# Edward-Sun/DIFUSCO

Measured on NVIDIA H100. Metric: TSP-500 graphs/sec, 50-step categorical denoise, higher is better.
Workload: dtype f32 (3-term bf16 split on wgmma, fp32 accumulate)

## Files before the change

difusco_b200/_cabi.py:

```python
import ctypes as C
import os

import numpy as np

HERE = os.path.dirname(os.path.abspath(__file__))
LIB_PATH = os.path.join(HERE, "libdifusco_b200.so")

DFB_OK, DFB_E_INVALID, DFB_E_CUDA, DFB_E_UNSUPPORTED, DFB_E_NOMEM = 0, -1, -2, -3, -4
CATEGORICAL, GAUSSIAN = 0, 1
EDGE_IMPL_TC, EDGE_IMPL_FP32, EDGE_IMPL_TC1 = 0, 1, 2
AGGREGATION = {"sum": 0, "mean": 1, "max": 2}

SYMBOLS = [
    "dfb_abi_version", "dfb_create", "dfb_destroy", "dfb_last_error", "dfb_set_aggregation",
    "dfb_set_edge_impl", "dfb_load_weights", "dfb_prepare_graph", "dfb_set_points",
    "dfb_encoder_forward", "dfb_denoise_step", "dfb_denoise", "dfb_denoise_record", "dfb_denoise_host",
    "dfb_launch_count", "dfb_profile_begin", "dfb_profile_end", "dfb_debug_edge_gemm", "dfb_debug_gnn_layer",
    "dfb_debug_phase_cycles", "dfb_debug_watchdog", "dfb_knn_graph", "dfb_set_graph_capture",
    "dfb_set_phase_timing", "dfb_tsp_merge_sparse", "dfb_tsp_merge_order", "dfb_two_opt", "dfb_write_heatmap_txt",
]

_lib = None


def lib():
  global _lib
  if _lib is not None:
    return _lib
  if not os.path.exists(LIB_PATH):
    raise RuntimeError(
        f"{LIB_PATH} not found: build it with `python -m difusco_b200.build` "
        "(difusco_b200 has no fallback path; the CUDA library is the product)")
  L = C.CDLL(LIB_PATH)
  vp, i32, i64, u64, f32 = C.c_void_p, C.c_int, C.c_int64, C.c_uint64, C.c_float
  L.dfb_abi_version.restype = i32
  L.dfb_create.argtypes = [C.POINTER(vp), i32]
  L.dfb_destroy.argtypes = [vp]
  L.dfb_last_error.argtypes = [vp]
  L.dfb_last_error.restype = C.c_char_p
  L.dfb_set_aggregation.argtypes = [vp, i32]
  L.dfb_set_edge_impl.argtypes = [vp, i32]
  L.dfb_load_weights.argtypes = [vp, i32, i32, i32, i32, i32, C.POINTER(C.c_char_p), C.POINTER(vp),
                                 C.POINTER(i64)]
  L.dfb_prepare_graph.argtypes = [vp, vp, i64, i64, i32, vp]
  L.dfb_set_points.argtypes = [vp, vp, vp]
  L.dfb_encoder_forward.argtypes = [vp, vp, f32, vp, vp]
  L.dfb_denoise_step.argtypes = [vp, i32, vp, f32, C.POINTER(f32), i32, vp, u64, i32, vp, vp, vp, vp]
  L.dfb_denoise.argtypes = [vp, i32, vp, i32, C.POINTER(C.c_int32), C.POINTER(f32),
                            C.POINTER(C.c_int32), vp, u64, vp]
  L.dfb_denoise_record.argtypes = [vp, i32, vp, i32, C.POINTER(C.c_int32), C.POINTER(f32), C.POINTER(C.c_int32), vp,
                                   u64, i32, C.POINTER(C.c_int32), vp, vp, vp, vp]
  L.dfb_denoise_host.argtypes = [vp, i32, vp, vp, i64, i64, i32, vp, i32, C.POINTER(C.c_int32),
                                 C.POINTER(f32), C.POINTER(C.c_int32), u64, vp, vp]
  L.dfb_launch_count.argtypes = [vp]
  L.dfb_launch_count.restype = i64
  L.dfb_profile_begin.argtypes = [vp]
  L.dfb_profile_end.argtypes = [vp, C.POINTER(C.c_double), C.POINTER(i64)]
  L.dfb_debug_edge_gemm.argtypes = [vp, i32, vp, vp, vp]
  L.dfb_debug_gnn_layer.argtypes = [vp, i32, f32, vp, vp, vp]
  L.dfb_debug_phase_cycles.argtypes = [vp, C.POINTER(C.c_uint64)]
  L.dfb_debug_watchdog.argtypes = [vp, C.POINTER(C.c_int)]
  L.dfb_set_graph_capture.argtypes = [vp, i32]
  L.dfb_set_phase_timing.argtypes = [vp, i32]
  L.dfb_knn_graph.argtypes = [vp, vp, i64, i32, i64, vp, vp]
  L.dfb_tsp_merge_sparse.argtypes = [vp, i64, vp, vp, i64, i32, vp, C.POINTER(i64)]
  L.dfb_tsp_merge_order.argtypes = [i64, vp, i64, vp, C.POINTER(i64)]
  L.dfb_two_opt.argtypes = [vp, vp, i64, vp, i64, i64, C.POINTER(i64), vp]
  L.dfb_write_heatmap_txt.argtypes = [C.c_char_p, i64, vp]
  for name in SYMBOLS:
    fn = getattr(L, name)
    if fn.restype is C.c_int and name not in ("dfb_abi_version",):
      fn.restype = i32
  _lib = L
  return L


class DfbError(RuntimeError):
  pass


def _raise(code, msg):
  msg = msg.decode() if isinstance(msg, bytes) else msg
  if code == DFB_E_INVALID:
    raise ValueError(msg)
  if code == DFB_E_UNSUPPORTED:
    raise NotImplementedError(msg)
  if code == DFB_E_NOMEM:
    raise MemoryError(msg)
  raise DfbError(msg)


MERGE_COMPLETE, MERGE_INCOMPLETE, MERGE_AMBIGUOUS = 0, 1, 2


def tsp_merge_sparse(points, heat, edge_index, mode=0):
  points = np.ascontiguousarray(points, dtype=np.float64)
  heat = np.ascontiguousarray(heat, dtype=np.float32).reshape(-1)
  edge_index = np.ascontiguousarray(edge_index, dtype=np.int64)
  n = points.shape[0]
  if edge_index.ndim != 2 or edge_index.shape[0] != 2 or edge_index.shape[1] != heat.shape[0]:
    raise ValueError("edge_index must be (2, E) with one heat value per edge")
  tour = np.empty(n + 1, dtype=np.int64)
  it = C.c_int64(0)
  rc = lib().dfb_tsp_merge_sparse(points.ctypes.data, n, heat.ctypes.data, edge_index.ctypes.data, heat.shape[0],
                                  int(mode), tour.ctypes.data, C.byref(it))
  if rc < 0:
    _raise(rc, "dfb_tsp_merge_sparse: invalid argument (n >= 3, indices inside [0, n), mode 0/1)")
  return rc, tour, it.value


def tsp_merge_order(n, order):
  order = np.ascontiguousarray(order, dtype=np.int64).reshape(-1)
  tour = np.empty(n + 1, dtype=np.int64)
  it = C.c_int64(0)
# ... 96 lines not shown
  def denoise(self, diffusion, xt_ptr, t1, consts, last, uniforms_ptr=None, seed=0, stream=0):
    steps, t1a, ca, la = self._sched_arrays(t1, consts, last)
    self._ck(lib().dfb_denoise(self._h, diffusion, xt_ptr, steps, t1a, ca, la, uniforms_ptr,
                               int(seed) & 0xFFFFFFFFFFFFFFFF, stream))

  def denoise_record(self, diffusion, xt_ptr, t1, consts, last, record_steps, rec_xt_ptr=None, rec_p_ptr=None,
                     rec_out_ptr=None, uniforms_ptr=None, seed=0, stream=0):
    steps, t1a, ca, la = self._sched_arrays(t1, consts, last)
    n_rec = len(record_steps)
    ra = (C.c_int32 * max(n_rec, 1))(*[int(x) for x in record_steps])
    self._ck(lib().dfb_denoise_record(self._h, diffusion, xt_ptr, steps, t1a, ca, la, uniforms_ptr,
                                      int(seed) & 0xFFFFFFFFFFFFFFFF, n_rec, ra, rec_xt_ptr, rec_p_ptr, rec_out_ptr,
                                      stream))

  def denoise_host(self, diffusion, points_ptr, edge_index_ptr, num_nodes, num_edges, gn_segments, xt0_ptr,
                   t1, consts, last, seed, heatmap_ptr, stream=0):
    steps, t1a, ca, la = self._sched_arrays(t1, consts, last)
    self._ck(lib().dfb_denoise_host(self._h, diffusion, points_ptr, edge_index_ptr, num_nodes, num_edges,
                                    gn_segments, xt0_ptr, steps, t1a, ca, la,
                                    int(seed) & 0xFFFFFFFFFFFFFFFF, heatmap_ptr, stream))

  def two_opt(self, points, tours, max_iterations, stream=0):
    points = np.ascontiguousarray(points, dtype=np.float64)
    tours = np.array(tours, dtype=np.int64, order="C", copy=True)
    if tours.ndim != 2 or tours.shape[1] != points.shape[0] + 1:
      raise ValueError("tours must be (batch, n + 1)")
    it = C.c_int64(0)
    self._ck(lib().dfb_two_opt(self._h, points.ctypes.data, points.shape[0], tours.ctypes.data, tours.shape[0],
                               int(max_iterations), C.byref(it), stream))
    return tours, it.value

  def knn_graph(self, points_ptr, num_nodes, k, node_offset, edge_index_ptr, stream=0):
    self._ck(lib().dfb_knn_graph(self._h, points_ptr, int(num_nodes), int(k), int(node_offset), edge_index_ptr, stream))

  def launch_count(self):
    return int(lib().dfb_launch_count(self._h))

  def profile_begin(self):
    self._ck(lib().dfb_profile_begin(self._h))

  def profile_end(self):
    ms, n = C.c_double(0), C.c_int64(0)
    self._ck(lib().dfb_profile_end(self._h, C.byref(ms), C.byref(n)))
    return ms.value, n.value

  def set_graph_capture(self, enabled):
    self._ck(lib().dfb_set_graph_capture(self._h, int(bool(enabled))))

  def debug_watchdog(self):
    out = (C.c_int * 4)()
    lib().dfb_debug_watchdog(self._h, out)
    return [int(x) for x in out]

  def set_phase_timing(self, enabled):
    self._ck(lib().dfb_set_phase_timing(self._h, int(bool(enabled))))

  def debug_phase_cycles(self):
    out = (C.c_uint64 * 32)()
    self._ck(lib().dfb_debug_phase_cycles(self._h, out))
    return [int(x) for x in out]

  def debug_edge_gemm(self, layer, e_in_ptr, acc_out_ptr, stream=0):
    self._ck(lib().dfb_debug_edge_gemm(self._h, layer, e_in_ptr, acc_out_ptr, stream))

  def debug_gnn_layer(self, layer, t, h_ptr, e_ptr, stream=0):
    self._ck(lib().dfb_debug_gnn_layer(self._h, int(layer), float(t), h_ptr, e_ptr, stream))
```

difusco_b200/csrc/dfb_api.cu:

```cuda
#include <cuda_runtime.h>
#include <math.h>
#include <stdio.h>
#include <stdlib.h>
#include <string.h>

#include <map>
#include <string>
#include <vector>

#include "../../include/difusco_b200.h"
#include "common.cuh"
#include "edge_layer_fp32.cuh"
#include "edge_layer_tc.cuh"
#include "kernels_small.cuh"
#include "knn.cuh"
#include "tsp_decode.cuh"

using namespace dfb;

static std::string g_create_error;

struct DevBuf {
  void* p = nullptr;
  size_t cap = 0;
// ... 938 lines not shown
  if (ms) *ms = tot;
  if (n) *n = (int64_t)(ctx->ev_used / 2);
  ctx->profiling = false;
  ctx->ev_used = 0;
  return DFB_OK;
}

extern "C" int dfb_debug_edge_gemm(dfb_ctx* ctx, int layer, const float* e_in, float* acc_out, void* stream_) {
  if (!ctx) return DFB_E_INVALID;
  cudaStream_t st = (cudaStream_t)stream_;
  CK(ctx, cudaSetDevice(ctx->device));
  if (!ctx->graph_ready) FAIL(ctx, DFB_E_INVALID, "dfb_prepare_graph must be called first");
  if (layer < 0 || layer >= ctx->L) FAIL(ctx, DFB_E_INVALID, "layer out of range");
  if (tc_launch_edge_layer(&ctx->tc, layer, const_cast<float*>(e_in), (const float*)ctx->uvab.p,
                           (float*)ctx->partials.p, ctx->g, ctx->layers[layer], nullptr, 0, 0, nullptr, ctx->lut, AGG_SUM,
                           edge_impl(ctx).nwg, false, acc_out, st))
    FAIL(ctx, DFB_E_CUDA, "tensor-core edge layer: %s", ctx->tc.err.c_str());
  ctx->launches++;
  return DFB_OK;
}

extern "C" int dfb_debug_gnn_layer(dfb_ctx* ctx, int layer, float t, float* h, float* e, void* stream_) {
  if (!ctx) return DFB_E_INVALID;
  cudaStream_t st = (cudaStream_t)stream_;
  CK(ctx, cudaSetDevice(ctx->device));
  if (!ctx->graph_ready) FAIL(ctx, DFB_E_INVALID, "dfb_prepare_graph must be called first");
  if (layer < 0 || layer >= ctx->L) FAIL(ctx, DFB_E_INVALID, "layer %d out of range for %d layers", layer, ctx->L);
  if (!is_device_ptr(h) || !is_device_ptr(e)) FAIL(ctx, DFB_E_INVALID, "h and e must be device pointers");
  int slot;
  int r = stage_acquire(ctx, &slot);
  if (r) return r;
  ctx->h_tvals[slot][0] = t;
  r = compute_tvecs(ctx, slot, 1, st);
  if (r) return r;
  CK(ctx, cudaEventRecord(ctx->stage_ev[slot], st));
  return run_layer(ctx, layer, h, e, nullptr, (const float*)ctx->tvec.p + (size_t)layer * H, 0, nullptr, st);
}

extern "C" int dfb_debug_phase_cycles(dfb_ctx* ctx, unsigned long long* out) {
  if (!ctx || !out) return DFB_E_INVALID;
  CK(ctx, cudaSetDevice(ctx->device));
  CK(ctx, cudaDeviceSynchronize());
  CK(ctx, cudaMemcpy(out, ctx->tc.phase_cycles, 32 * sizeof(unsigned long long), cudaMemcpyDeviceToHost));
  CK(ctx, cudaMemset(ctx->tc.phase_cycles, 0, 32 * sizeof(unsigned long long)));
  return DFB_OK;
}

extern "C" int dfb_debug_watchdog(dfb_ctx* ctx, int* out) {
  if (!ctx || !out || !ctx->tc.error_host) return DFB_E_INVALID;
  for (int i = 0; i < 4; ++i) out[i] = ((volatile int*)ctx->tc.error_host)[i];
  return DFB_OK;
}

extern "C" int dfb_knn_graph(dfb_ctx* ctx, const double* points, int64_t num_nodes, int k, int64_t node_offset,
                             int64_t* edge_index, void* stream_) {
  if (!ctx) return DFB_E_INVALID;
  cudaStream_t st = (cudaStream_t)stream_;
  CK(ctx, cudaSetDevice(ctx->device));
  if (num_nodes < 1 || k < 1 || k > num_nodes) FAIL(ctx, DFB_E_INVALID, "bad kNN size N=%lld K=%d", (long long)num_nodes, k);
  if ((size_t)num_nodes * sizeof(double) > 200 * 1024) FAIL(ctx, DFB_E_UNSUPPORTED, "kNN graph: N=%lld exceeds the shared-memory brute-force limit (25600)", (long long)num_nodes);
  const size_t smem = (size_t)num_nodes * sizeof(double) + (size_t)(num_nodes + 31) / 32 * sizeof(unsigned);
  if (!is_device_ptr(edge_index)) FAIL(ctx, DFB_E_INVALID, "edge_index must be a device pointer");
  const double* dp = points;
  if (!is_device_ptr(points)) {
    for (int64_t i = 0; i < 2 * num_nodes; ++i)
      if (!std::isfinite(points[i])) FAIL(ctx, DFB_E_INVALID, "kNN graph: non-finite coordinate of node %lld", (long long)(i / 2));
    ENS(ctx, ctx->d_points, (size_t)num_nodes * 2 * sizeof(double));
    CK(ctx, cudaMemcpyAsync(ctx->d_points.p, points, (size_t)num_nodes * 2 * sizeof(double), cudaMemcpyHostToDevice, st));
    dp = (const double*)ctx->d_points.p;
  }
  CK(ctx, cudaFuncSetAttribute(k_knn_bruteforce, cudaFuncAttributeMaxDynamicSharedMemorySize, (int)smem));
  k_knn_bruteforce<<<(int)num_nodes, 256, smem, st>>>(dp, (int)num_nodes, k, (long long*)edge_index, (long long)node_offset);
  CKL(ctx);
  return DFB_OK;
}

extern "C" int dfb_tsp_merge_sparse(const double* points, int64_t n, const float* heat, const int64_t* edge_index, int64_t E,
                                    int mode, int64_t* tour, int64_t* merge_iterations) {
  if (!points || !heat || !edge_index || !tour || !merge_iterations || n < 3 || n > 0x7fffffff / 2 || E < 0 || (mode != 0 && mode != 1))
    return DFB_E_INVALID;
  int r = tspmerge::merge_sparse(points, (int)n, heat, edge_index, E, mode, tour, merge_iterations);
  return r < 0 ? DFB_E_INVALID : r;
}

extern "C" int dfb_tsp_merge_order(int64_t n, const int64_t* order, int64_t count, int64_t* tour, int64_t* merge_iterations) {
  if (!order || !tour || !merge_iterations || n < 3 || n > 0x7fffffff / 2 || count < 0) return DFB_E_INVALID;
  int r = tspmerge::merge_order((int)n, order, count, tour, merge_iterations);
  return r < 0 ? DFB_E_INVALID : r;
}

extern "C" int dfb_two_opt(dfb_ctx* ctx, const double* points, int64_t n, int64_t* tours, int64_t batch, int64_t max_iterations,
                           int64_t* iterations_out, void* stream_) {
  if (!ctx) return DFB_E_INVALID;
  cudaStream_t st = (cudaStream_t)stream_;
  CK(ctx, cudaSetDevice(ctx->device));
  if (!points || !tours || !iterations_out) FAIL(ctx, DFB_E_INVALID, "two_opt: null argument");
  if (n < 3 || n > 46340 || batch < 1 || batch > 65535) FAIL(ctx, DFB_E_INVALID, "two_opt: bad size n=%lld batch=%lld (n in [3, 46340], batch in [1, 65535])", (long long)n, (long long)batch);
  const int N = (int)n, B = (int)batch;
  bool finite = true;
  for (int64_t k = 0; k < batch * (n + 1); ++k) {
    if (tours[k] < 0 || tours[k] >= n) FAIL(ctx, DFB_E_INVALID, "two_opt: tour entry %lld out of range", (long long)tours[k]);
    finite = finite && std::isfinite(points[2 * tours[k]]) && std::isfinite(points[2 * tours[k] + 1]);
  }
  if (!finite) {
    *iterations_out = 0;
    return DFB_OK;
// ... 79 lines not shown
```

difusco_b200/csrc/edge_layer_tc.cuh:

```cuda
#pragma once
#include <cuda.h>
#include <cuda_bf16.h>
#include <cuda_runtime.h>

#include <stdlib.h>

#include <string>

#include "common.cuh"
#include "edge_layer_fp32.cuh"

namespace dfb {

constexpr int WG_ROWS = 64;
constexpr int TC_KCH = 64;
constexpr int TC_B_BYTES = 256 * 128;
constexpr int TC_A_CHUNK = WG_ROWS * 128;
constexpr int TC_A_BYTES = 8 * TC_A_CHUNK;
constexpr int CONV_BATCH = 16;
constexpr int E4_BATCH = 16;

constexpr int W_LO_ROWS = H;
constexpr int W_MAT_ROWS = 2 * W_LO_ROWS;
constexpr int W_LAYER_ROWS = 6 * W_MAT_ROWS;
__host__ __device__ constexpr int w_row_C(int l) { return l * W_LAYER_ROWS; }
__host__ __device__ constexpr int w_row_O(int l) { return w_row_C(l) + W_MAT_ROWS; }
__host__ __device__ constexpr int w_row_UVAB(int l) { return w_row_C(l) + 2 * W_MAT_ROWS; }
__host__ __device__ constexpr int w_row_embed(int L, int which) { return L * W_LAYER_ROWS + which * W_MAT_ROWS; }
__host__ __device__ constexpr int w_arena_rows(int L) { return w_row_embed(L, 2); }

template <int NWG>
struct TcCfg {
  static_assert(NWG == 1 || NWG == 2, "one or two consumer warpgroups");
  static constexpr int TILE = NWG * WG_ROWS;
  static constexpr int THREADS = (NWG + 1) * 128;
  static constexpr int NSTAGE = (NWG == 1) ? 3 : 2;
  static constexpr int OFF_B = NWG * TC_A_BYTES;
  static constexpr int OFF_PRM = OFF_B + NSTAGE * TC_B_BYTES;
  static constexpr int OFF_ROW = OFF_PRM + 6 * H * 4;
  static constexpr int OFF_SRC = OFF_ROW + TILE * 4;
  static constexpr int OFF_BAR = OFF_SRC + TILE * 8;
  static constexpr int SMEM_BYTES = OFF_BAR + 2 * NSTAGE * 8;
  static constexpr int SMEM_ALLOC = SMEM_BYTES + 1024;
  static_assert(SMEM_ALLOC <= 232448, "shared memory budget (227 KB per block)");
};

struct TcParams {
  float* e;
  const float* uvab;
  float* partials;
  GraphDev g;
  LayerParams lp;
  const float* tvec;
  const float* xt_lut;
  const float* lut;
  const float* zero_row;
  float* debug_acc;
  const float* lin_in;
  float* lin_out;
  const float* lin_bias;
  int lin_rows;
  int lin_nb;
  int lin_w_row;
  int* error_flag;
  unsigned long long* phase_cycles;
  int write_e, e_zero, agg_mode;
  int w_row_base;
  int n_tiles;
};

__device__ __forceinline__ uint32_t smem_u32(const void* p) { return (uint32_t)__cvta_generic_to_shared(p); }

__device__ __forceinline__ void mbar_init(uint64_t* bar, uint32_t count) {
  asm volatile("mbarrier.init.shared::cta.b64 [%0], %1;" ::"r"(smem_u32(bar)), "r"(count) : "memory");
}
__device__ __forceinline__ void mbar_arrive(uint64_t* bar) {
  asm volatile("mbarrier.arrive.shared::cta.b64 _, [%0];" ::"r"(smem_u32(bar)) : "memory");
}
__device__ __forceinline__ void mbar_arrive_expect_tx(uint64_t* bar, uint32_t bytes) {
  asm volatile("mbarrier.arrive.expect_tx.shared::cta.b64 _, [%0], %1;" ::"r"(smem_u32(bar)), "r"(bytes) : "memory");
}
__device__ __forceinline__ void mbar_wait(uint64_t* bar, uint32_t parity, int* error_flag, int code) {
  const uint32_t addr = smem_u32(bar);
  uint32_t ok = 0;
#pragma unroll 1
  for (uint32_t spin = 0;; ++spin) {
    asm volatile(
        "{\n .reg .pred p;\n mbarrier.try_wait.parity.shared::cta.b64 p, [%1], %2, %3;\n selp.u32 %0, 1, 0, p;\n}"
        : "=r"(ok)
        : "r"(addr), "r"(parity), "r"(20000u)
        : "memory");
    if (ok) return;
    if (spin > 400000u) {
      if (error_flag) {
        error_flag[1] = (int)blockIdx.x;
        error_flag[2] = (int)parity;
        error_flag[3] = (int)threadIdx.x;
        atomicExch(error_flag, code);
      }
      __threadfence_system();
      __trap();
    }
  }
}
__device__ __forceinline__ void tma_load_2d(uint32_t dst, const CUtensorMap* map, uint64_t* bar, int c0, int c1) {
  asm volatile(
      "cp.async.bulk.tensor.2d.shared::cluster.global.mbarrier::complete_tx::bytes [%0], [%1, {%3, %4}], [%2];"
      ::"r"(dst), "l"(reinterpret_cast<uint64_t>(map)), "r"(smem_u32(bar)), "r"(c0), "r"(c1)
      : "memory");
}
__device__ __forceinline__ void fence_proxy_async() { asm volatile("fence.proxy.async.shared::cta;" ::: "memory"); }

__device__ __forceinline__ uint64_t wgmma_desc_sw128(uint32_t smem_addr) {
  return (uint64_t)((smem_addr >> 4) & 0x3fffu) | (1ull << 16) | (64ull << 32) | (1ull << 62);
}
__device__ __forceinline__ void wgmma_fence() { asm volatile("wgmma.fence.sync.aligned;" ::: "memory"); }
__device__ __forceinline__ void wgmma_commit() { asm volatile("wgmma.commit_group.sync.aligned;" ::: "memory"); }
template <int N>
__device__ __forceinline__ void wgmma_wait() { asm volatile("wgmma.wait_group.sync.aligned %0;" ::"n"(N) : "memory"); }
__device__ __forceinline__ void acc_fence(float (&d)[128]) {
#pragma unroll
  for (int i = 0; i < 128; ++i) asm volatile("" : "+f"(d[i])::"memory");
}
__device__ __forceinline__ void wgmma_bf16(float (&d)[128], uint64_t da, uint64_t db, uint32_t scale_d) {
  asm volatile(
      "{\n .reg .pred p;\n setp.ne.b32 p, %130, 0;\n"
      "wgmma.mma_async.sync.aligned.m64n256k16.f32.bf16.bf16 "
      "{%0, %1, %2, %3, %4, %5, %6, %7, %8, %9, %10, %11, %12, %13, %14, %15, "
      "%16, %17, %18, %19, %20, %21, %22, %23, %24, %25, %26, %27, %28, %29, %30, %31, "
      "%32, %33, %34, %35, %36, %37, %38, %39, %40, %41, %42, %43, %44, %45, %46, %47, "
      "%48, %49, %50, %51, %52, %53, %54, %55, %56, %57, %58, %59, %60, %61, %62, %63, "
      "%64, %65, %66, %67, %68, %69, %70, %71, %72, %73, %74, %75, %76, %77, %78, %79, "
      "%80, %81, %82, %83, %84, %85, %86, %87, %88, %89, %90, %91, %92, %93, %94, %95, "
      "%96, %97, %98, %99, %100, %101, %102, %103, %104, %105, %106, %107, %108, %109, %110, %111, "
      "%112, %113, %114, %115, %116, %117, %118, %119, %120, %121, %122, %123, %124, %125, %126, %127}, "
      "%128, %129, p, 1, 1, 0, 0;\n}"
      : "+f"(d[0]), "+f"(d[1]), "+f"(d[2]), "+f"(d[3]), "+f"(d[4]), "+f"(d[5]), "+f"(d[6]), "+f"(d[7]),
        "+f"(d[8]), "+f"(d[9]), "+f"(d[10]), "+f"(d[11]), "+f"(d[12]), "+f"(d[13]), "+f"(d[14]), "+f"(d[15]),
        "+f"(d[16]), "+f"(d[17]), "+f"(d[18]), "+f"(d[19]), "+f"(d[20]), "+f"(d[21]), "+f"(d[22]), "+f"(d[23]),
        "+f"(d[24]), "+f"(d[25]), "+f"(d[26]), "+f"(d[27]), "+f"(d[28]), "+f"(d[29]), "+f"(d[30]), "+f"(d[31]),
        "+f"(d[32]), "+f"(d[33]), "+f"(d[34]), "+f"(d[35]), "+f"(d[36]), "+f"(d[37]), "+f"(d[38]), "+f"(d[39]),
        "+f"(d[40]), "+f"(d[41]), "+f"(d[42]), "+f"(d[43]), "+f"(d[44]), "+f"(d[45]), "+f"(d[46]), "+f"(d[47]),
        "+f"(d[48]), "+f"(d[49]), "+f"(d[50]), "+f"(d[51]), "+f"(d[52]), "+f"(d[53]), "+f"(d[54]), "+f"(d[55]),
        "+f"(d[56]), "+f"(d[57]), "+f"(d[58]), "+f"(d[59]), "+f"(d[60]), "+f"(d[61]), "+f"(d[62]), "+f"(d[63]),
        "+f"(d[64]), "+f"(d[65]), "+f"(d[66]), "+f"(d[67]), "+f"(d[68]), "+f"(d[69]), "+f"(d[70]), "+f"(d[71]),
        "+f"(d[72]), "+f"(d[73]), "+f"(d[74]), "+f"(d[75]), "+f"(d[76]), "+f"(d[77]), "+f"(d[78]), "+f"(d[79]),
        "+f"(d[80]), "+f"(d[81]), "+f"(d[82]), "+f"(d[83]), "+f"(d[84]), "+f"(d[85]), "+f"(d[86]), "+f"(d[87]),
        "+f"(d[88]), "+f"(d[89]), "+f"(d[90]), "+f"(d[91]), "+f"(d[92]), "+f"(d[93]), "+f"(d[94]), "+f"(d[95]),
        "+f"(d[96]), "+f"(d[97]), "+f"(d[98]), "+f"(d[99]), "+f"(d[100]), "+f"(d[101]), "+f"(d[102]), "+f"(d[103]),
        "+f"(d[104]), "+f"(d[105]), "+f"(d[106]), "+f"(d[107]), "+f"(d[108]), "+f"(d[109]), "+f"(d[110]), "+f"(d[111]),
        "+f"(d[112]), "+f"(d[113]), "+f"(d[114]), "+f"(d[115]), "+f"(d[116]), "+f"(d[117]), "+f"(d[118]), "+f"(d[119]),
        "+f"(d[120]), "+f"(d[121]), "+f"(d[122]), "+f"(d[123]), "+f"(d[124]), "+f"(d[125]), "+f"(d[126]), "+f"(d[127])
      : "l"(da), "l"(db), "r"(scale_d));
}

__device__ __forceinline__ float sigmoid_mufu(float x) {
  float t, r;
  asm("ex2.approx.ftz.f32 %0, %1;" : "=f"(t) : "f"(-1.4426950408889634f * x));
  asm("rcp.approx.ftz.f32 %0, %1;" : "=f"(r) : "f"(1.0f + t));
  return r;
}
__device__ __forceinline__ void split4(float4 x, uint2& hi, uint2& lo) {
// ... 10 lines not shown
  __nv_bfloat162 h = __floats2bfloat162_rn(a, b);
  const float2 f = __bfloat1622float2(h);
  __nv_bfloat162 l = __floats2bfloat162_rn(a - f.x, b - f.y);
  hi = *reinterpret_cast<uint32_t*>(&h);
  lo = *reinterpret_cast<uint32_t*>(&l);
}
__device__ __forceinline__ uint32_t sw128_off(int r, int j) {
  return (uint32_t)((r >> 3) * 1024 + (r & 7) * 128 + ((j ^ (r & 7)) << 4));
}
__device__ __forceinline__ float quad_sum(float v) {
  v += __shfl_xor_sync(0xffffffffu, v, 1);
  return v + __shfl_xor_sync(0xffffffffu, v, 2);
}
__device__ __forceinline__ void swap_row_halves(float (&d)[128]) {
#pragma unroll
  for (int j = 0; j < 32; ++j) {
    const float x0 = d[4 * j], x1 = d[4 * j + 1];
    d[4 * j] = d[4 * j + 2];
    d[4 * j + 1] = d[4 * j + 3];
    d[4 * j + 2] = x0;
    d[4 * j + 3] = x1;
  }
}

enum {
  PH_TILES = 0,
  PH_TOTAL,
  PH_CONVERT,
  PH_G1_WAIT,
  PH_G1_MMA,
  PH_E1,
  PH_REDUCE,
  PH_LN,
  PH_G2_WAIT,
  PH_G2_MMA,
  PH_E4,
  PH_COUNT
};

template <int NWG, bool LIN, bool TIMED = false>
__device__ __forceinline__ void edge_layer_wg_body(const CUtensorMap& wmap, const TcParams& P) {
  using Cfg = TcCfg<NWG>;
  constexpr int NSTAGE = Cfg::NSTAGE;
  extern __shared__ unsigned char smem_raw[];
  unsigned char* smem = smem_raw + ((1024u - (smem_u32(smem_raw) & 1023u)) & 1023u);
  float* prm = reinterpret_cast<float*>(smem + Cfg::OFF_PRM);
  int* s_row = reinterpret_cast<int*>(smem + Cfg::OFF_ROW);
  const float** s_src = reinterpret_cast<const float**>(smem + Cfg::OFF_SRC);
  uint64_t* full = reinterpret_cast<uint64_t*>(smem + Cfg::OFF_BAR);
  uint64_t* empty = full + NSTAGE;

  const int warp = threadIdx.x >> 5, lane = threadIdx.x & 31;
  constexpr bool lin = LIN;
  const int loads_per_tile = (P.write_e ? 16 : 8) * NWG;

  if (threadIdx.x == 0) {
    for (int s = 0; s < NSTAGE; ++s) {
      mbar_init(&full[s], 1);
      mbar_init(&empty[s], 4);
    }
    asm volatile("fence.mbarrier_init.release.cluster;" ::: "memory");
    fence_proxy_async();
  }
  for (int i = threadIdx.x; i < H; i += Cfg::THREADS) {
    prm[i] = P.lp.ln_e_g[i];
    prm[H + i] = P.lp.ln_e_b[i];
    prm[2 * H + i] = P.tvec ? P.tvec[i] : 0.0f;
    prm[3 * H + i] = P.lp.ln_o_g[i];
    prm[4 * H + i] = P.lp.ln_o_b[i];
    prm[5 * H + i] = P.lp.b_O[i];
  }
  __syncthreads();
  const uint32_t smem_base = smem_u32(smem);

  if (warp >= 4 * NWG) {
    if constexpr (NWG == 2) asm volatile("setmaxnreg.dec.sync.aligned.u32 40;" ::: "memory");
    if (warp == 4 * NWG && lane == 0) {
      uint32_t u = 0;
      for (int tile = blockIdx.x; tile < P.n_tiles; tile += gridDim.x) {
        for (int i = 0; i < loads_per_tile; ++i, ++u) {
          const int s = u % NSTAGE;
          mbar_wait(&empty[s], ((u / NSTAGE) & 1) ^ 1, P.error_flag, 1);
          mbar_arrive_expect_tx(&full[s], TC_B_BYTES);
          const int row = (lin ? P.lin_w_row + (P.lin_nb == 4 ? (tile & 3) : 0) * W_MAT_ROWS
                               : P.w_row_base + (i >= 8 * NWG ? w_row_O(0) - w_row_C(0) : 0)) +
                          (i & 1) * W_LO_ROWS;
          tma_load_2d(smem_base + Cfg::OFF_B + s * TC_B_BYTES, &wmap, &full[s], ((i >> 1) & 3) * TC_KCH, row);
        }
      }
    }
    return;
  }

  if constexpr (NWG == 2) asm volatile("setmaxnreg.inc.sync.aligned.u32 232;" ::: "memory");
  const int wg = warp >> 2, wi = warp & 3, tid = threadIdx.x & 127;
  const int t4 = lane & 3;
  const int lr0 = wi * 16 + (lane >> 2);
  unsigned char* a_reg = smem + wg * TC_A_BYTES;
  const uint32_t a_base = smem_base + wg * TC_A_BYTES;
  float* msg = reinterpret_cast<float*>(a_reg);
  int* w_row = s_row + wg * WG_ROWS;
  const float** w_src = s_src + wg * WG_ROWS;
  auto wg_bar = [&] { asm volatile("bar.sync %0, 128;" ::"r"(1 + wg) : "memory"); };
  const int n_rows = lin ? P.lin_rows : P.g.E;
  uint32_t u = 0;
  float acc[128];

  auto turn_wait = [&] {
    if constexpr (NWG == 2) asm volatile("bar.sync %0, 256;" ::"r"(3 + wg) : "memory");
  };
  auto turn_pass = [&] {
    if constexpr (NWG == 2) asm volatile("bar.arrive %0, 256;" ::"r"(4 - wg) : "memory");
  };
  if (wg == 1) turn_pass();

  uint32_t t_mark = 0, t_start = 0;
  if constexpr (TIMED) t_start = t_mark = (uint32_t)clock();
  auto record = [&](int slot, uint32_t v) {
    if constexpr (TIMED) {
      if (tid == 0) atomicAdd(P.phase_cycles + slot, (unsigned long long)v);
    }
  };
  auto mark = [&](int slot) {
    if constexpr (TIMED) {
      const uint32_t now = (uint32_t)clock();
      record(slot, now - t_mark);
      t_mark = now;
    }
  };

  auto gemm = [&](int wait_slot, int mma_slot) {
    uint32_t waited = 0;
    turn_wait();
    if constexpr (TIMED) t_mark = (uint32_t)clock();
    acc_fence(acc);
    wgmma_fence();
    int s_prev = 0;
#pragma unroll
    for (int i = 0; i < 8; ++i, ++u) {
      const int s = u % NSTAGE;
      uint32_t w0 = 0;
      if constexpr (TIMED) w0 = (uint32_t)clock();
      mbar_wait(&full[s], (u / NSTAGE) & 1, P.error_flag, 2);
      if constexpr (TIMED) waited += (uint32_t)clock() - w0;
      const uint32_t b = smem_base + Cfg::OFF_B + s * TC_B_BYTES;
      const uint32_t ahi = a_base + (i >> 1) * 2 * TC_A_CHUNK, alo = ahi + TC_A_CHUNK;
#pragma unroll
      for (int ks = 0; ks < 4; ++ks) {
        const uint64_t db = wgmma_desc_sw128(b + ks * 32);
        wgmma_bf16(acc, wgmma_desc_sw128(ahi + ks * 32), db, (i | ks) ? 1u : 0u);
        if ((i & 1) == 0) wgmma_bf16(acc, wgmma_desc_sw128(alo + ks * 32), db, 1u);
      }
      wgmma_commit();
      if (i > 0) {
        wgmma_wait<1>();
        __syncwarp();
        if (lane == 0) mbar_arrive(&empty[s_prev]);
      }
      s_prev = s;
    }
    wgmma_wait<0>();
    acc_fence(acc);
    __syncwarp();
    if (lane == 0) mbar_arrive(&empty[s_prev]);
    turn_pass();
    if constexpr (TIMED) {
      const uint32_t now = (uint32_t)clock();
      record(wait_slot, waited);
      record(mma_slot, now - t_mark - waited);
      t_mark = now;
    }
  };

  for (int tile = blockIdx.x; tile < P.n_tiles; tile += gridDim.x) {
    record(PH_TILES, 1);
    const int row_tile = (lin && P.lin_nb == 4) ? (tile >> 2) : tile;
    const int s_base = row_tile * Cfg::TILE + wg * WG_ROWS;
    if (tid < WG_ROWS) {
      const int s = s_base + tid;
      const float* src = P.zero_row;
      int rw = -1;
      if (s < n_rows && lin) {
        src = P.lin_in + (size_t)s * H;
      } else if (s < n_rows) {
        rw = P.g.row[s];
        if (P.e_zero) src = P.zero_row;
        else if (P.xt_lut) src = P.lut + ((P.xt_lut[P.g.perm ? P.g.perm[s] : s] != 0.0f) ? H : 0);
        else src = P.e + (size_t)s * H;
      }
      w_row[tid] = rw;
      w_src[tid] = src;
    }
    wg_bar();

#pragma unroll 1
    for (int it0 = 0; it0 < 32; it0 += CONV_BATCH) {
      float4 x[CONV_BATCH];
#pragma unroll
      for (int q = 0; q < CONV_BATCH; ++q) {
        const int item = (it0 + q) * 128 + tid;
        x[q] = __ldcg(reinterpret_cast<const float4*>(w_src[item >> 6]) + (item & 63));
      }
#pragma unroll
      for (int q = 0; q < CONV_BATCH; ++q) {
        const int item = (it0 + q) * 128 + tid;
        const int rr = item >> 6, k4 = item & 63;
        uint2 hi, lo;
        split4(x[q], hi, lo);
        const uint32_t off = (k4 >> 4) * 2 * TC_A_CHUNK + sw128_off(rr, (k4 & 15) >> 1) + (k4 & 1) * 8;
        *reinterpret_cast<uint2*>(a_reg + off) = hi;
        *reinterpret_cast<uint2*>(a_reg + off + TC_A_CHUNK) = lo;
      }
    }
    fence_proxy_async();
    wg_bar();
    mark(PH_CONVERT);
    gemm(PH_G1_WAIT, PH_G1_MMA);

    const int sa = s_base + lr0, sb = sa + 8;
    const bool va = sa < n_rows, vb = sb < n_rows;
    if (lin || P.debug_acc) {
      const int nb = (lin && P.lin_nb == 4) ? (tile & 3) : 0;
      const int ostride = lin ? P.lin_nb * H : H;
      float* out = lin ? P.lin_out + nb * H : P.debug_acc;
#pragma unroll
      for (int h = 0; h < 2; ++h) {
        const int s = h ? sb : sa;
        if (!(h ? vb : va)) continue;
#pragma unroll
// ... 97 lines not shown
      mean = quad_sum(sum) * (1.0f / H);
      q = 0.f;
#pragma unroll
      for (int j = 0; j < 32; ++j) {
        const float d0 = acc[4 * j] - mean, d1 = acc[4 * j + 1] - mean;
        q = fmaf(d0, d0, fmaf(d1, d1, q));
      }
      rstd = rsqrtf(quad_sum(q) * (1.0f / H) + LN_EPS);
      const int r = lr0 + 8 * h;
#pragma unroll
      for (int j = 0; j < 32; ++j) {
        const int c = 8 * j + 2 * t4;
        const float2 g = *reinterpret_cast<const float2*>(prm + 3 * H + c);
        const float2 b = *reinterpret_cast<const float2*>(prm + 4 * H + c);
        const float z0 = fmaf((acc[4 * j] - mean) * rstd, g.x, b.x);
        const float z1 = fmaf((acc[4 * j + 1] - mean) * rstd, g.y, b.y);
        uint32_t hi, lo;
        split2(z0 * sigmoid_mufu(z0), z1 * sigmoid_mufu(z1), hi, lo);
        const uint32_t off = (j >> 3) * 2 * TC_A_CHUNK + sw128_off(r, j & 7) + 4 * t4;
        *reinterpret_cast<uint32_t*>(a_reg + off) = hi;
        *reinterpret_cast<uint32_t*>(a_reg + off + TC_A_CHUNK) = lo;
      }
      swap_row_halves(acc);
    }
    fence_proxy_async();
    wg_bar();
    mark(PH_LN);
    gemm(PH_G2_WAIT, PH_G2_MMA);

#pragma unroll
    for (int h = 0; h < 2; ++h) {
      if (!(h ? vb : va)) continue;
      const float* src = h ? src_b : src_a;
      float* dst = P.e + (size_t)(h ? sb : sa) * H;
#pragma unroll
      for (int j0 = 0; j0 < 32; j0 += E4_BATCH) {
        float2 ein[E4_BATCH];
#pragma unroll
        for (int q = 0; q < E4_BATCH; ++q) ein[q] = __ldcg(reinterpret_cast<const float2*>(src + 8 * (j0 + q) + 2 * t4));
#pragma unroll
        for (int q = 0; q < E4_BATCH; ++q) {
          const int j = j0 + q, c = 8 * j + 2 * t4;
          const float2 bo = *reinterpret_cast<const float2*>(prm + 5 * H + c);
          __stcg(reinterpret_cast<float2*>(dst + c),
                 make_float2((ein[q].x + acc[4 * j + 2 * h]) + bo.x, (ein[q].y + acc[4 * j + 2 * h + 1]) + bo.y));
        }
      }
    }
    mark(PH_E4);
  }
  if constexpr (TIMED) record(PH_TOTAL, (uint32_t)clock() - t_start);
}

__global__ void __launch_bounds__(TcCfg<2>::THREADS, 1)
k_edge_layer_wg2(const __grid_constant__ CUtensorMap wmap, const TcParams P) {
  edge_layer_wg_body<2, false>(wmap, P);
}
__global__ void __launch_bounds__(TcCfg<2>::THREADS, 1)
k_edge_layer_wg2_timed(const __grid_constant__ CUtensorMap wmap, const TcParams P) {
  edge_layer_wg_body<2, false, true>(wmap, P);
}
__global__ void __launch_bounds__(TcCfg<1>::THREADS, 1)
k_edge_layer_wg1(const __grid_constant__ CUtensorMap wmap, const TcParams P) {
  edge_layer_wg_body<1, false>(wmap, P);
}
__global__ void __launch_bounds__(TcCfg<2>::THREADS, 1)
k_linear_wg2(const __grid_constant__ CUtensorMap wmap, const TcParams P) {
  edge_layer_wg_body<2, true>(wmap, P);
}

struct TcState {
  std::string err;
  int num_sms = 0;
  CUtensorMap wmap;
  bool bound = false;
  float* zero_row = nullptr;
  int* error_flag = nullptr;
  int* error_host = nullptr;
  unsigned long long* phase_cycles = nullptr;

  TcState() = default;
  TcState(const TcState&) = delete;
  TcState& operator=(const TcState&) = delete;
  ~TcState() {
    if (zero_row) cudaFree(zero_row);
    if (error_host) cudaFreeHost(error_host);
    if (phase_cycles) cudaFree(phase_cycles);
  }
};

typedef CUresult (*PFN_encodeTiled)(CUtensorMap*, CUtensorMapDataType, cuuint32_t, void*, const cuuint64_t*,
                                    const cuuint64_t*, const cuuint32_t*, const cuuint32_t*, CUtensorMapInterleave,
                                    CUtensorMapSwizzle, CUtensorMapL2promotion, CUtensorMapFloatOOBfill);

inline int tc_init(TcState* st, int num_sms) {
  st->num_sms = num_sms;
  cudaError_t e = cudaFuncSetAttribute(k_edge_layer_wg2, cudaFuncAttributeMaxDynamicSharedMemorySize, TcCfg<2>::SMEM_ALLOC);
  if (e == cudaSuccess)
    e = cudaFuncSetAttribute(k_edge_layer_wg2_timed, cudaFuncAttributeMaxDynamicSharedMemorySize, TcCfg<2>::SMEM_ALLOC);
  if (e == cudaSuccess)
    e = cudaFuncSetAttribute(k_edge_layer_wg1, cudaFuncAttributeMaxDynamicSharedMemorySize, TcCfg<1>::SMEM_ALLOC);
  if (e == cudaSuccess)
    e = cudaFuncSetAttribute(k_linear_wg2, cudaFuncAttributeMaxDynamicSharedMemorySize, TcCfg<2>::SMEM_ALLOC);
  if (e != cudaSuccess) {
    st->err = std::string("cudaFuncSetAttribute: ") + cudaGetErrorString(e);
    return -2;
  }
  if ((e = cudaMalloc(&st->zero_row, H * sizeof(float))) != cudaSuccess ||
      (e = cudaMemset(st->zero_row, 0, H * sizeof(float))) != cudaSuccess ||
      (e = cudaMalloc(&st->phase_cycles, 32 * sizeof(unsigned long long))) != cudaSuccess ||
      (e = cudaMemset(st->phase_cycles, 0, 32 * sizeof(unsigned long long))) != cudaSuccess ||
      (e = cudaHostAlloc(&st->error_host, 4 * sizeof(int), cudaHostAllocMapped)) != cudaSuccess ||
      (e = cudaHostGetDevicePointer((void**)&st->error_flag, st->error_host, 0)) != cudaSuccess) {
    st->err = std::string("tc_init alloc: ") + cudaGetErrorString(e);
    return -2;
  }
  return 0;
}

inline int tc_bind_weights(TcState* st, const uint16_t* arena, int L) {
  void* fn = nullptr;
  cudaDriverEntryPointQueryResult qres;
  cudaError_t e = cudaGetDriverEntryPoint("cuTensorMapEncodeTiled", &fn, cudaEnableDefault, &qres);
  if (e != cudaSuccess || !fn || qres != cudaDriverEntryPointSuccess) {
    st->err = "cuTensorMapEncodeTiled entry point not available";
    cudaGetLastError();
    return -2;
  }
  cuuint64_t gdim[2] = {(cuuint64_t)H, (cuuint64_t)w_arena_rows(L)};
  cuuint64_t gstride[1] = {(cuuint64_t)H * sizeof(uint16_t)};
  cuuint32_t box[2] = {(cuuint32_t)TC_KCH, 256u};
  cuuint32_t estr[2] = {1u, 1u};
  CUresult r = ((PFN_encodeTiled)fn)(&st->wmap, CU_TENSOR_MAP_DATA_TYPE_BFLOAT16, 2, (void*)arena, gdim,
                                     gstride, box, estr, CU_TENSOR_MAP_INTERLEAVE_NONE, CU_TENSOR_MAP_SWIZZLE_128B,
                                     CU_TENSOR_MAP_L2_PROMOTION_L2_256B, CU_TENSOR_MAP_FLOAT_OOB_FILL_NONE);
  if (r != CUDA_SUCCESS) {
    st->err = "cuTensorMapEncodeTiled failed with CUresult " + std::to_string((int)r);
    return -2;
  }
  st->bound = true;
  return 0;
}

template <int NWG>
inline int tc_launch(TcState* st, void (*kernel)(CUtensorMap, TcParams), TcParams& P, int rows, int nb,
                     cudaStream_t stream) {
  if (!st->bound) {
    st->err = "weights not bound";
    return -1;
  }
  P.zero_row = st->zero_row; P.error_flag = st->error_flag; P.phase_cycles = st->phase_cycles;
  P.n_tiles = nb * ((rows + TcCfg<NWG>::TILE - 1) / TcCfg<NWG>::TILE);
  const int grid = P.n_tiles < st->num_sms ? P.n_tiles : st->num_sms;
  kernel<<<grid, TcCfg<NWG>::THREADS, TcCfg<NWG>::SMEM_ALLOC, stream>>>(st->wmap, P);
  const cudaError_t err = cudaGetLastError();
  if (err == cudaSuccess) return 0;
  st->err = std::string("launch: ") + cudaGetErrorString(err);
  return -2;
}

inline int tc_launch_edge_layer(TcState* st, int l, float* e, const float* uvab, float* partials, const GraphDev& g,
                                const LayerParams& lp, const float* tvec, int write_e, int e_zero, const float* xt_lut,
                                const float* lut, int agg_mode, int nwg, bool timed, float* debug_acc,
                                cudaStream_t stream) {
  TcParams P{};
  P.e = e; P.uvab = uvab; P.partials = partials; P.g = g; P.lp = lp; P.tvec = tvec;
  P.xt_lut = xt_lut; P.lut = lut; P.debug_acc = debug_acc;
  P.write_e = debug_acc ? 0 : write_e;
  P.e_zero = e_zero; P.agg_mode = agg_mode;
  P.w_row_base = w_row_C(l);
  if (nwg == 1) return tc_launch<1>(st, k_edge_layer_wg1, P, g.E, 1, stream);
  return tc_launch<2>(st, timed && !debug_acc ? k_edge_layer_wg2_timed : k_edge_layer_wg2, P, g.E, 1, stream);
}

inline int tc_launch_linear(TcState* st, const float* in, float* out, const float* bias, int rows, int nb, int w_row,
                            cudaStream_t stream) {
  TcParams P{};
  P.lin_in = in; P.lin_out = out; P.lin_bias = bias; P.lin_rows = rows; P.lin_nb = nb; P.lin_w_row = w_row;
  P.lp.ln_e_g = P.lp.ln_e_b = P.lp.ln_o_g = P.lp.ln_o_b = P.lp.b_O = st->zero_row;
  return tc_launch<2>(st, k_linear_wg2, P, rows, nb, stream);
}

}
```

include/difusco_b200.h:

```cpp
#ifndef DIFUSCO_B200_H_
#define DIFUSCO_B200_H_

#include <stdint.h>

#ifdef __cplusplus
extern "C" {
#endif

#define DFB_ABI_VERSION 2

enum {
  DFB_OK = 0,
  DFB_E_INVALID = -1,
  DFB_E_CUDA = -2,
  DFB_E_UNSUPPORTED = -3,
  DFB_E_NOMEM = -4
};

enum { DFB_TASK_TSP = 0, DFB_TASK_MIS = 1 };
enum { DFB_DIFFUSION_CATEGORICAL = 0, DFB_DIFFUSION_GAUSSIAN = 1 };
enum { DFB_EDGE_IMPL_TC = 0, DFB_EDGE_IMPL_FP32 = 1, DFB_EDGE_IMPL_TC1 = 2 };

typedef struct dfb_ctx dfb_ctx;

// ... 16 lines not shown

int dfb_set_points(dfb_ctx* ctx, const float* points, void* stream);

int dfb_encoder_forward(dfb_ctx* ctx, const float* xt, float t, float* out, void* stream);

int dfb_denoise_step(dfb_ctx* ctx, int diffusion_type, const float* xt_in, float t,
                     const float* consts, int last, const float* uniforms, uint64_t seed,
                     int step_index, float* xt_out, float* p_out, float* net_out, void* stream);

int dfb_denoise(dfb_ctx* ctx, int diffusion_type, float* xt, int steps, const int32_t* t1,
                const float* consts, const int32_t* last_flags, const float* uniforms,
                uint64_t seed, void* stream);

int dfb_denoise_record(dfb_ctx* ctx, int diffusion_type, float* xt, int steps, const int32_t* t1,
                       const float* consts, const int32_t* last_flags, const float* uniforms, uint64_t seed,
                       int n_record, const int32_t* record_steps, float* rec_xt, float* rec_p, float* rec_out,
                       void* stream);

int dfb_set_graph_capture(dfb_ctx* ctx, int enabled);

int dfb_denoise_host(dfb_ctx* ctx, int diffusion_type, const float* points,
                     const int64_t* edge_index, int64_t num_nodes, int64_t num_edges,
                     int gn_segments, const float* xt0, int steps, const int32_t* t1,
                     const float* consts, const int32_t* last_flags, uint64_t seed,
                     float* heatmap_out, void* stream);

int dfb_knn_graph(dfb_ctx* ctx, const double* points, int64_t num_nodes, int k, int64_t node_offset,
                  int64_t* edge_index, void* stream);

int dfb_tsp_merge_sparse(const double* points, int64_t n, const float* heat, const int64_t* edge_index, int64_t E,
                         int mode, int64_t* tour, int64_t* merge_iterations);
int dfb_tsp_merge_order(int64_t n, const int64_t* order, int64_t count, int64_t* tour, int64_t* merge_iterations);

int dfb_two_opt(dfb_ctx* ctx, const double* points, int64_t n, int64_t* tours, int64_t batch, int64_t max_iterations,
                int64_t* iterations_out, void* stream);

int dfb_write_heatmap_txt(const char* path, int64_t n, const double* matrix);

int64_t dfb_launch_count(const dfb_ctx* ctx);

int dfb_profile_begin(dfb_ctx* ctx);
int dfb_profile_end(dfb_ctx* ctx, double* edge_kernel_ms, int64_t* edge_kernel_launches);

int dfb_debug_edge_gemm(dfb_ctx* ctx, int layer, const float* e_in, float* acc_out, void* stream);

int dfb_debug_gnn_layer(dfb_ctx* ctx, int layer, float t, float* h, float* e, void* stream);

int dfb_debug_phase_cycles(dfb_ctx* ctx, unsigned long long* out);

int dfb_set_phase_timing(dfb_ctx* ctx, int enabled);

int dfb_debug_watchdog(dfb_ctx* ctx, int* out);

#ifdef __cplusplus
}
#endif
#endif
```

Baseline: 20.77.

## Pair edge-layer CTAs into 2-CTA clusters sharing weight tiles via TMA multicast

Runs the 2-warpgroup edge-layer kernel as 2-CTA clusters. Each CTA's producer TMA-loads half of every 256-row weight B tile and multicasts it to both CTAs, so each CTA issues half the weight traffic from L2. Consumer warps now release a stage to both CTAs' empty barriers, and the producer drains the peer's releases before exiting. The grid is sized from the occupancy-reported maximum active clusters and the tile count is padded to even, which adds cross-CTA coupling and lockstep stalls between paired CTAs.

```diff
diff --git a/difusco_b200/_cabi.py b/difusco_b200/_cabi.py
--- a/difusco_b200/_cabi.py
+++ b/difusco_b200/_cabi.py
@@ -16,7 +16,7 @@
     "dfb_set_edge_impl", "dfb_load_weights", "dfb_prepare_graph", "dfb_set_points",
     "dfb_encoder_forward", "dfb_denoise_step", "dfb_denoise", "dfb_denoise_record", "dfb_denoise_host",
     "dfb_launch_count", "dfb_profile_begin", "dfb_profile_end", "dfb_debug_edge_gemm", "dfb_debug_gnn_layer",
-    "dfb_debug_phase_cycles", "dfb_debug_watchdog", "dfb_knn_graph", "dfb_set_graph_capture",
+    "dfb_debug_phase_cycles", "dfb_debug_watchdog", "dfb_debug_edge_grid", "dfb_knn_graph", "dfb_set_graph_capture",
     "dfb_set_phase_timing", "dfb_tsp_merge_sparse", "dfb_tsp_merge_order", "dfb_two_opt", "dfb_write_heatmap_txt",
 ]
 
@@ -60,6 +60,7 @@
   L.dfb_debug_gnn_layer.argtypes = [vp, i32, f32, vp, vp, vp]
   L.dfb_debug_phase_cycles.argtypes = [vp, C.POINTER(C.c_uint64)]
   L.dfb_debug_watchdog.argtypes = [vp, C.POINTER(C.c_int)]
+  L.dfb_debug_edge_grid.argtypes = [vp, C.POINTER(C.c_int)]
   L.dfb_set_graph_capture.argtypes = [vp, i32]
   L.dfb_set_phase_timing.argtypes = [vp, i32]
   L.dfb_knn_graph.argtypes = [vp, vp, i64, i32, i64, vp, vp]
@@ -262,6 +263,11 @@
     lib().dfb_debug_watchdog(self._h, out)
     return [int(x) for x in out]
 
+  def debug_edge_grid(self):
+    out = (C.c_int * 2)()
+    self._ck(lib().dfb_debug_edge_grid(self._h, out))
+    return [int(x) for x in out]
+
   def set_phase_timing(self, enabled):
     self._ck(lib().dfb_set_phase_timing(self._h, int(bool(enabled))))
 
diff --git a/difusco_b200/csrc/dfb_api.cu b/difusco_b200/csrc/dfb_api.cu
--- a/difusco_b200/csrc/dfb_api.cu
+++ b/difusco_b200/csrc/dfb_api.cu
@@ -1014,6 +1014,13 @@
   return DFB_OK;
 }
 
+extern "C" int dfb_debug_edge_grid(dfb_ctx* ctx, int* out) {
+  if (!ctx || !out) return DFB_E_INVALID;
+  out[0] = ctx->tc.pair_clusters;
+  out[1] = 2 * ctx->tc.pair_clusters;
+  return DFB_OK;
+}
+
 extern "C" int dfb_knn_graph(dfb_ctx* ctx, const double* points, int64_t num_nodes, int k, int64_t node_offset,
                              int64_t* edge_index, void* stream_) {
   if (!ctx) return DFB_E_INVALID;
diff --git a/difusco_b200/csrc/edge_layer_tc.cuh b/difusco_b200/csrc/edge_layer_tc.cuh
--- a/difusco_b200/csrc/edge_layer_tc.cuh
+++ b/difusco_b200/csrc/edge_layer_tc.cuh
@@ -15,6 +15,8 @@
 constexpr int WG_ROWS = 64;
 constexpr int TC_KCH = 64;
 constexpr int TC_B_BYTES = 256 * 128;
+constexpr int TC_B_HALF_ROWS = 128;
+constexpr int TC_B_HALF = TC_B_HALF_ROWS * 128;
 constexpr int TC_A_CHUNK = WG_ROWS * 128;
 constexpr int TC_A_BYTES = 8 * TC_A_CHUNK;
 constexpr int CONV_BATCH = 16;
@@ -108,6 +110,27 @@
       "cp.async.bulk.tensor.2d.shared::cluster.global.mbarrier::complete_tx::bytes [%0], [%1, {%3, %4}], [%2];"
       ::"r"(dst), "l"(reinterpret_cast<uint64_t>(map)), "r"(smem_u32(bar)), "r"(c0), "r"(c1)
       : "memory");
+}
+__device__ __forceinline__ void tma_load_2d_pair(uint32_t dst, const CUtensorMap* map, uint64_t* bar, int c0, int c1) {
+  asm volatile(
+      "cp.async.bulk.tensor.2d.shared::cluster.global.mbarrier::complete_tx::bytes.multicast::cluster"
+      " [%0], [%1, {%3, %4}], [%2], %5;"
+      ::"r"(dst), "l"(reinterpret_cast<uint64_t>(map)), "r"(smem_u32(bar)), "r"(c0), "r"(c1), "h"((uint16_t)0x3)
+      : "memory");
+}
+__device__ __forceinline__ uint32_t cluster_ctarank() {
+  uint32_t r;
+  asm volatile("mov.u32 %0, %%cluster_ctarank;" : "=r"(r));
+  return r;
+}
+__device__ __forceinline__ void mbar_arrive_peer(uint64_t* bar) {
+  asm volatile(
+      "{\n .reg .b32 r, a;\n mov.u32 r, %%cluster_ctarank;\n xor.b32 r, r, 1;\n mapa.shared::cluster.u32 a, %0, r;\n"
+      " mbarrier.arrive.release.cta.shared::cluster.b64 _, [a];\n}" ::"r"(smem_u32(bar))
+      : "memory");
+}
+__device__ __forceinline__ void cluster_sync() {
+  asm volatile("barrier.cluster.arrive.release.aligned;\n barrier.cluster.wait.acquire.aligned;" ::: "memory");
 }
 __device__ __forceinline__ void fence_proxy_async() { asm volatile("fence.proxy.async.shared::cta;" ::: "memory"); }
 
@@ -224,12 +247,13 @@
 
   const int warp = threadIdx.x >> 5, lane = threadIdx.x & 31;
   constexpr bool lin = LIN;
+  constexpr bool PAIR = NWG == 2 && !LIN;
   const int loads_per_tile = (P.write_e ? 16 : 8) * NWG;
 
   if (threadIdx.x == 0) {
     for (int s = 0; s < NSTAGE; ++s) {
       mbar_init(&full[s], 1);
-      mbar_init(&empty[s], 4);
+      mbar_init(&empty[s], PAIR ? 8 : 4);
     }
     asm volatile("fence.mbarrier_init.release.cluster;" ::: "memory");
     fence_proxy_async();
@@ -242,7 +266,8 @@
     prm[4 * H + i] = P.lp.ln_o_b[i];
     prm[5 * H + i] = P.lp.b_O[i];
   }
-  __syncthreads();
+  if constexpr (PAIR) cluster_sync();
+  else __syncthreads();
   const uint32_t smem_base = smem_u32(smem);
 
   if (warp >= 4 * NWG) {
@@ -257,8 +282,19 @@
           const int row = (lin ? P.lin_w_row + (P.lin_nb == 4 ? (tile & 3) : 0) * W_MAT_ROWS
                                : P.w_row_base + (i >= 8 * NWG ? w_row_O(0) - w_row_C(0) : 0)) +
                           (i & 1) * W_LO_ROWS;
-          tma_load_2d(smem_base + Cfg::OFF_B + s * TC_B_BYTES, &wmap, &full[s], ((i >> 1) & 3) * TC_KCH, row);
+          const uint32_t dst = smem_base + Cfg::OFF_B + s * TC_B_BYTES;
+          const int k0 = ((i >> 1) & 3) * TC_KCH;
+          if constexpr (PAIR) {
+            const uint32_t r = cluster_ctarank();
+            tma_load_2d_pair(dst + r * TC_B_HALF, &wmap, &full[s], k0, row + (int)r * TC_B_HALF_ROWS);
+          } else {
+            tma_load_2d(dst, &wmap, &full[s], k0, row);
+            tma_load_2d(dst + TC_B_HALF, &wmap, &full[s], k0, row + TC_B_HALF_ROWS);
+          }
         }
+      }
+      if constexpr (PAIR) {
+        for (int i = 0; i < NSTAGE; ++i, ++u) mbar_wait(&empty[u % NSTAGE], ((u / NSTAGE) & 1) ^ 1, P.error_flag, 3);
       }
     }
     return;
@@ -301,6 +337,11 @@
     }
   };
 
+  auto release = [&](int s) {
+    mbar_arrive(&empty[s]);
+    if constexpr (PAIR) mbar_arrive_peer(&empty[s]);
+  };
+
   auto gemm = [&](int wait_slot, int mma_slot) {
     uint32_t waited = 0;
     turn_wait();
@@ -327,14 +368,14 @@
       if (i > 0) {
         wgmma_wait<1>();
         __syncwarp();
-        if (lane == 0) mbar_arrive(&empty[s_prev]);
+        if (lane == 0) release(s_prev);
       }
       s_prev = s;
     }
     wgmma_wait<0>();
     acc_fence(acc);
     __syncwarp();
-    if (lane == 0) mbar_arrive(&empty[s_prev]);
+    if (lane == 0) release(s_prev);
     turn_pass();
     if constexpr (TIMED) {
       const uint32_t now = (uint32_t)clock();
@@ -345,8 +386,8 @@
   };
 
   for (int tile = blockIdx.x; tile < P.n_tiles; tile += gridDim.x) {
-    record(PH_TILES, 1);
     const int row_tile = (lin && P.lin_nb == 4) ? (tile >> 2) : tile;
+    record(PH_TILES, row_tile * Cfg::TILE < n_rows);
     const int s_base = row_tile * Cfg::TILE + wg * WG_ROWS;
     if (tid < WG_ROWS) {
       const int s = s_base + tid;
@@ -550,11 +591,11 @@
   if constexpr (TIMED) record(PH_TOTAL, (uint32_t)clock() - t_start);
 }
 
-__global__ void __launch_bounds__(TcCfg<2>::THREADS, 1)
+__global__ void __cluster_dims__(2, 1, 1) __launch_bounds__(TcCfg<2>::THREADS, 1)
 k_edge_layer_wg2(const __grid_constant__ CUtensorMap wmap, const TcParams P) {
   edge_layer_wg_body<2, false>(wmap, P);
 }
-__global__ void __launch_bounds__(TcCfg<2>::THREADS, 1)
+__global__ void __cluster_dims__(2, 1, 1) __launch_bounds__(TcCfg<2>::THREADS, 1)
 k_edge_layer_wg2_timed(const __grid_constant__ CUtensorMap wmap, const TcParams P) {
   edge_layer_wg_body<2, false, true>(wmap, P);
 }
@@ -570,6 +611,7 @@
 struct TcState {
   std::string err;
   int num_sms = 0;
+  int pair_clusters = 0;
   CUtensorMap wmap;
   bool bound = false;
   float* zero_row = nullptr;
@@ -604,6 +646,19 @@
     st->err = std::string("cudaFuncSetAttribute: ") + cudaGetErrorString(e);
     return -2;
   }
+  cudaLaunchConfig_t cfg = {};
+  cudaLaunchAttribute cl;
+  cl.id = cudaLaunchAttributeClusterDimension;
+  cl.val.clusterDim.x = 2; cl.val.clusterDim.y = 1; cl.val.clusterDim.z = 1;
+  cfg.gridDim = dim3(2 * num_sms); cfg.blockDim = dim3(TcCfg<2>::THREADS);
+  cfg.dynamicSmemBytes = TcCfg<2>::SMEM_ALLOC;
+  cfg.attrs = &cl; cfg.numAttrs = 1;
+  if ((e = cudaOccupancyMaxActiveClusters(&st->pair_clusters, k_edge_layer_wg2, &cfg)) != cudaSuccess ||
+      st->pair_clusters < 1) {
+    st->err = std::string("cudaOccupancyMaxActiveClusters: ") +
+              (e != cudaSuccess ? cudaGetErrorString(e) : "no 2-CTA cluster fits");
+    return -2;
+  }
   if ((e = cudaMalloc(&st->zero_row, H * sizeof(float))) != cudaSuccess ||
       (e = cudaMemset(st->zero_row, 0, H * sizeof(float))) != cudaSuccess ||
       (e = cudaMalloc(&st->phase_cycles, 32 * sizeof(unsigned long long))) != cudaSuccess ||
@@ -627,7 +682,7 @@
   }
   cuuint64_t gdim[2] = {(cuuint64_t)H, (cuuint64_t)w_arena_rows(L)};
   cuuint64_t gstride[1] = {(cuuint64_t)H * sizeof(uint16_t)};
-  cuuint32_t box[2] = {(cuuint32_t)TC_KCH, 256u};
+  cuuint32_t box[2] = {(cuuint32_t)TC_KCH, (cuuint32_t)TC_B_HALF_ROWS};
   cuuint32_t estr[2] = {1u, 1u};
   CUresult r = ((PFN_encodeTiled)fn)(&st->wmap, CU_TENSOR_MAP_DATA_TYPE_BFLOAT16, 2, (void*)arena, gdim,
                                      gstride, box, estr, CU_TENSOR_MAP_INTERLEAVE_NONE, CU_TENSOR_MAP_SWIZZLE_128B,
@@ -641,7 +696,7 @@
 }
 
 template <int NWG>
-inline int tc_launch(TcState* st, void (*kernel)(CUtensorMap, TcParams), TcParams& P, int rows, int nb,
+inline int tc_launch(TcState* st, void (*kernel)(CUtensorMap, TcParams), TcParams& P, int rows, int nb, bool pair,
                      cudaStream_t stream) {
   if (!st->bound) {
     st->err = "weights not bound";
@@ -649,7 +704,11 @@
   }
   P.zero_row = st->zero_row; P.error_flag = st->error_flag; P.phase_cycles = st->phase_cycles;
   P.n_tiles = nb * ((rows + TcCfg<NWG>::TILE - 1) / TcCfg<NWG>::TILE);
-  const int grid = P.n_tiles < st->num_sms ? P.n_tiles : st->num_sms;
+  int grid = P.n_tiles < st->num_sms ? P.n_tiles : st->num_sms;
+  if (pair) {
+    P.n_tiles = (P.n_tiles + 1) & ~1;
+    grid = 2 * (P.n_tiles / 2 < st->pair_clusters ? P.n_tiles / 2 : st->pair_clusters);
+  }
   kernel<<<grid, TcCfg<NWG>::THREADS, TcCfg<NWG>::SMEM_ALLOC, stream>>>(st->wmap, P);
   const cudaError_t err = cudaGetLastError();
   if (err == cudaSuccess) return 0;
@@ -667,8 +726,8 @@
   P.write_e = debug_acc ? 0 : write_e;
   P.e_zero = e_zero; P.agg_mode = agg_mode;
   P.w_row_base = w_row_C(l);
-  if (nwg == 1) return tc_launch<1>(st, k_edge_layer_wg1, P, g.E, 1, stream);
-  return tc_launch<2>(st, timed && !debug_acc ? k_edge_layer_wg2_timed : k_edge_layer_wg2, P, g.E, 1, stream);
+  if (nwg == 1) return tc_launch<1>(st, k_edge_layer_wg1, P, g.E, 1, false, stream);
+  return tc_launch<2>(st, timed && !debug_acc ? k_edge_layer_wg2_timed : k_edge_layer_wg2, P, g.E, 1, true, stream);
 }
 
 inline int tc_launch_linear(TcState* st, const float* in, float* out, const float* bias, int rows, int nb, int w_row,
@@ -676,7 +735,7 @@
   TcParams P{};
   P.lin_in = in; P.lin_out = out; P.lin_bias = bias; P.lin_rows = rows; P.lin_nb = nb; P.lin_w_row = w_row;
   P.lp.ln_e_g = P.lp.ln_e_b = P.lp.ln_o_g = P.lp.ln_o_b = P.lp.b_O = st->zero_row;
-  return tc_launch<2>(st, k_linear_wg2, P, rows, nb, stream);
-}
-
-}
+  return tc_launch<2>(st, k_linear_wg2, P, rows, nb, false, stream);
+}
+
+}
diff --git a/include/difusco_b200.h b/include/difusco_b200.h
--- a/include/difusco_b200.h
+++ b/include/difusco_b200.h
@@ -92,6 +92,8 @@
 
 int dfb_debug_watchdog(dfb_ctx* ctx, int* out);
 
+int dfb_debug_edge_grid(dfb_ctx* ctx, int* out);
+
 #ifdef __cplusplus
 }
 #endif
```

Measured after the change: 20.74 (median of 6 runs). About the same (-0.1%).
